# A-SHOJAEI/adverse-weather-semantic-segmentation-robustness-benchmark

Hardware: AMD Instinct MI355X
Metric: images/sec (1024x2048, 5 weather conds, ensemble eval) (higher is better)
Workload: dtype f32 (results float32; attention, gemm_1x1, winograd_3x3, segformer_head on 3xf16 split operands: 22-bit operands, f32 accumulate)

## Files before the change

### adverse_weather_semantic_segmentation_robustness_benchmark_amd/_native.py

```python
from __future__ import annotations

import ctypes as C
from pathlib import Path

import numpy as np
import torch

_PKG = Path(__file__).resolve().parent
LIB_PATH = _PKG / "libawseg_hip.so"

U8, I64 = 0, 1
COMBINE_WEIGHTED, COMBINE_MAXCONF, COMBINE_MEAN = 0, 1, 2
LOSS_CE, LOSS_FOCAL = 0, 1
ACT_NONE, ACT_RELU, ACT_GELU = 0, 1, 2
MAX_CLASSES = 32

c_i, c_i64, c_u64, c_f, c_d, c_p = C.c_int, C.c_int64, C.c_uint64, C.c_float, C.c_double, C.c_void_p

FOG_JOB = np.dtype([("image", "<i4"), ("_pad", "<i4"), ("beta", "<f8"), ("atmos", "<f8"), ("seed", "<u8")], align=True)
NIGHT_JOB = np.dtype([("image", "<i4"), ("_pad", "<i4"), ("brightness", "<f8"), ("intensity", "<f8"), ("seed", "<u8")], align=True)
PRIM_JOB = np.dtype([("image", "<i4"), ("prim_offset", "<i4"), ("prim_count", "<i4"), ("blur_ksize", "<i4"), ("intensity", "<f8")], align=True)
WEATHER_JOB = np.dtype([("kind", "<i4"), ("image", "<i4"), ("a", "<f8"), ("b", "<f8"), ("seed", "<u8"), ("prim_offset", "<i4"), ("prim_count", "<i4")], align=True)
WEATHER_CLEAN, WEATHER_FOG, WEATHER_RAIN, WEATHER_SNOW, WEATHER_NIGHT = 0, 1, 2, 3, 4
assert FOG_JOB.itemsize == 32 and NIGHT_JOB.itemsize == 32 and PRIM_JOB.itemsize == 24 and WEATHER_JOB.itemsize == 40
# ... 97 lines not shown
    "awseg_depth_eval_stats": (c_i, [c_p, c_p, c_i, c_i, c_i, c_i, c_i, c_p, c_p, c_f, c_p, c_p, c_i, c_p]),
    "awseg_ensemble_failure_stats": (c_i, [c_p, c_p, c_p, c_i64, c_i, c_i64, c_i, c_p, c_p, c_p, c_i, c_p, c_p, c_i, c_p]),
    "awseg_failure_stats": (c_i, [c_p, c_i64, c_i, c_i64, c_p, c_i, c_p, c_p, c_i, c_p]),
    "awseg_boundary_workspace": (c_i64, [c_i64, c_i, c_i, c_i, c_i]),
    "awseg_boundary_stats": (c_i, [c_p, c_p, c_i, c_i, c_i64, c_i, c_i, c_i, c_p, c_i, c_p, c_p, c_i, c_p, c_p, c_p]),
    "awseg_segment_workspace": (c_i64, [c_i64, c_i, c_i]),
    "awseg_segment_stats": (c_i, [c_p, c_p, c_i, c_i, c_i64, c_i, c_i, c_i, c_p, c_i, c_p, c_p, c_p, c_i, c_p, c_p, c_p, c_p, c_p]),
    "awseg_frame_iou_workspace": (c_i64, [c_i64, c_i, c_i64]),
    "awseg_frame_iou_counts": (c_i, [c_p, c_p, c_i, c_i, c_i64, c_i64, c_i, c_p, c_p, c_i64, c_p, c_p, c_p]),
    "awseg_bootstrap_counts": (c_i, [c_p, c_p, c_i64, c_i64, c_i64, c_i64, c_u64, c_i64, c_i64, c_p, c_p, c_p]),
    "awseg_change_strata": (c_i, [c_p, c_p, c_i, c_i64, c_i, c_i64, c_p, c_p, c_p, c_i, c_p, c_p, c_p]),
    "awseg_strata_workspace": (c_i64, [c_i64, c_i, c_i64, c_i]),
    "awseg_stratified_stats": (c_i, [c_p, c_p, c_i, c_i, c_p, c_i, c_p, c_i, c_p, c_i64, c_i64, c_i, c_p, c_p, c_i, c_p, c_p, c_p]),
    "awseg_image_quality_workspace": (c_i64, [c_i64, c_i, c_i64, c_i64]),
    "awseg_image_quality": (c_i, [c_p, c_p, c_i, c_i64, c_i, c_i64, c_i64, c_p, c_p, c_p, c_p, c_f, c_f, c_p, c_p, c_i, c_p, c_p, c_p]),
}

EXTENSION_SIGNATURES = {
    "awseg_restore_header_hash": (C.c_uint64, []),
    "awseg_dehaze_workspace": (c_i64, [c_i64, c_i64, c_i64]),
    "awseg_dehaze": (c_i, [c_p, c_i64, c_i, c_i64, c_i64, c_p, c_p, c_i, c_f, c_f, c_f, c_i, c_p, c_p, c_p, c_p, c_i, c_p, c_p]),
    "awseg_dehaze_guided_workspace": (c_i64, [c_i64, c_i64, c_i64]),
    "awseg_dehaze_guided": (c_i, [c_p, c_i64, c_i, c_i64, c_i64, c_p, c_p, c_i, c_f, c_f, c_f, c_i, c_f, c_p, c_p, c_p, c_p, c_p, c_p, c_i,
                                  c_p, c_p]),
    "awseg_relight_workspace": (c_i64, [c_i64, c_i, c_i]),
    "awseg_relight": (c_i, [c_p, c_i64, c_i, c_i64, c_i64, c_p, c_p, c_i, c_i, c_f, c_f, c_i, c_p, c_p, c_p, c_p, c_i, c_p, c_p]),
    "awseg_deocclude_workspace": (c_i64, [c_i64, c_i64, c_i64]),
    "awseg_deocclude": (c_i, [c_p, c_i64, c_i, c_i64, c_i64, c_p, c_p, c_i, c_f, c_f, c_i, c_p, c_p, c_p, c_p, c_i, c_p, c_p]),
    "awseg_weather_estimate_workspace": (c_i64, [c_i64]),
    "awseg_weather_estimate": (c_i, [c_p, c_i64, c_i, c_i64, c_i64, c_p, c_p, c_i, c_f, c_f, c_f, c_f, c_f, c_f, c_p, c_p, c_p, c_p, c_i,
                                     c_p, c_p]),
}


class AwsegError(RuntimeError):
    pass


_lib = None


def lib() -> C.CDLL:
    global _lib
    if _lib is None:
        if not LIB_PATH.exists():
            raise AwsegError(
                f"{LIB_PATH} is missing: build it with `python -m "
                "adverse_weather_semantic_segmentation_robustness_benchmark_amd.csrc.build` "
                "(there is no CPU fallback for the HIP hot path)")
        handle = C.CDLL(str(LIB_PATH))
        for table in (SIGNATURES, EXTENSION_SIGNATURES):
            for name, (res, args) in table.items():
                fn = getattr(handle, name)
                fn.restype, fn.argtypes = res, args
        header = LIB_PATH.parent.parent / "include" / "awseg.h"
        built = int(handle.awseg_header_hash())
        if built and header.exists():
            from .csrc.build import header_hash
            if built != header_hash():
                raise AwsegError(f"{LIB_PATH} was built from another include/awseg.h than the one beside it (ABI drift): rebuild it with "
                                 "`python -m adverse_weather_semantic_segmentation_robustness_benchmark_amd.csrc.build`")
        extension = header.with_name("awseg_restore.h")
        built = int(handle.awseg_restore_header_hash())
        if built and extension.exists():
            from .csrc.build import RESTORE_HEADER, header_hash
            if built != header_hash(RESTORE_HEADER):
                raise AwsegError(f"{LIB_PATH} was built from another include/awseg_restore.h than the one beside it (ABI drift): rebuild "
                                 "it with `python -m adverse_weather_semantic_segmentation_robustness_benchmark_amd.csrc.build`")
        _lib = handle
    return _lib


def check(rc: int, what: str) -> None:
    if rc != 0:
        msg = lib().awseg_error_string(rc)
        raise AwsegError(f"{what} failed with code {rc}: {msg.decode() if msg else '?'}")


launch_hook = None


def call(name: str, *args) -> None:
    fn = getattr(lib(), name)
    rc = fn(*args) if launch_hook is None else launch_hook(name, lambda: fn(*args), args)
    check(rc, name)


def try_call(name: str, *args, allow=(-2,)) -> int:
    fn = getattr(lib(), name)
    rc = fn(*args) if launch_hook is None else launch_hook(name, lambda: fn(*args), args)
    if rc != 0 and rc not in allow:
        check(rc, name)
    return rc


def ptr(t):
    if t is None:
        return None
    if not t.is_cuda:
        raise AwsegError("awseg kernels take device (HIP) tensors only; got a CPU tensor — no CPU fallback exists")
    if not t.is_contiguous():
# ... 49 lines not shown
```

### adverse_weather_semantic_segmentation_robustness_benchmark_amd/csrc/build.py

```python
from __future__ import annotations

import os
import shutil
import subprocess
import sys
from concurrent.futures import ThreadPoolExecutor
from pathlib import Path

CSRC = Path(__file__).resolve().parent
PKG = CSRC.parent
LIB = PKG / "libawseg_hip.so"
SOURCES = ["core.hip", "metrics.hip", "weather.hip", "loss.hip", "heads.hip", "backbone.hip", "depth.hip", "wino.hip", "gemm.hip", "attn.hip", "gemm_split.hip", "gemm_split3.hip", "wino_split.hip", "depthfuse.hip", "mixffn.hip", "dwtrain.hip", "bntrain.hip", "smallops.hip", "calib.hip", "consistency.hip", "deptheval.hip", "failure.hip", "boundary.hip", "bootstrap.hip", "strata.hip", "quality.hip", "segments.hip", "weightgrid.hip", "dehaze.hip", "dehaze_guided.hip", "relight.hip", "deocclude.hip", "estimate.hip"]
ARCH = "gfx950"
HEADER = PKG.parent / "include" / "awseg.h"
RESTORE_HEADER = PKG.parent / "include" / "awseg_restore.h"


def header_hash(path: Path = HEADER) -> int:
    import hashlib
    return int(hashlib.sha256(path.read_bytes()).hexdigest()[:15], 16)


EXTRA_FLAGS = {"attn.hip": ["-DAWSEG_ATTN_SPLIT_WAVES=" + os.environ.get("AWSEG_ATTN_SPLIT_WAVES", "2")], "wino.hip": ["-fno-slp-vectorize"], "wino_split.hip": ["-fno-slp-vectorize"],
               "core.hip": ["-DAWSEG_HEADER_HASH=0x%xULL" % header_hash()],
               "dehaze.hip": ["-DAWSEG_RESTORE_HEADER_HASH=0x%xULL" % header_hash(RESTORE_HEADER)]}


def hipcc() -> str:
    for cand in (os.environ.get("HIPCC"), "/opt/rocm/bin/hipcc", shutil.which("hipcc")):
        if cand and Path(cand).exists():
            return cand
    raise RuntimeError("hipcc not found (need ROCm's hipcc to build libawseg_hip.so)")


def _flags():
    return [f"--offload-arch={ARCH}", "-O3", "-std=c++17", "-fPIC", "-ffp-contract=off",
            "-fvisibility=hidden", "-Wall", "-Wno-unused-function", "-Wno-inline-asm"]


STAMP = PKG / "libawseg_hip.flags"


def _flag_stamp() -> str:
    return repr((_flags(), sorted(EXTRA_FLAGS.items()), SOURCES))


def needs_build() -> bool:
    if not LIB.exists():
        return True
    if not STAMP.exists() or STAMP.read_text() != _flag_stamp():
        return True
    t = LIB.stat().st_mtime
    deps = [CSRC / s for s in SOURCES] + sorted(CSRC.glob("*.h")) + [HEADER, RESTORE_HEADER]
    return any(d.stat().st_mtime > t for d in deps)


def build(force: bool = False, verbose: bool = False) -> Path:
    if not force and not needs_build():
        return LIB
    cc = hipcc()
    objdir = CSRC / "build"
    objdir.mkdir(exist_ok=True)

    def compile_one(src):
        obj = objdir / (Path(src).stem + ".o")
        cmd = [cc, *_flags(), *EXTRA_FLAGS.get(src, []), "-c", str(CSRC / src), "-o", str(obj)]
        if verbose:
            print(" ".join(cmd))
        subprocess.check_call(cmd)
        return obj

    with ThreadPoolExecutor(max_workers=min(4, len(SOURCES))) as ex:
        objs = list(ex.map(compile_one, SOURCES))
    tmp = LIB.with_suffix(".so.tmp")
    rocm_lib = str(Path(cc).resolve().parent.parent / "lib")
    subprocess.check_call([cc, f"--offload-arch={ARCH}", "-shared", "-fPIC", "-o", str(tmp), *map(str, objs),
                           f"-L{rocm_lib}", "-lhipblaslt", f"-Wl,-rpath,{rocm_lib}"])
    os.replace(tmp, LIB)
    STAMP.write_text(_flag_stamp())
    return LIB


if __name__ == "__main__":
    print(build(force="--force" in sys.argv, verbose=True))
```

### adverse_weather_semantic_segmentation_robustness_benchmark_amd/models/fused.py

```python
from __future__ import annotations

import contextlib
import os
from typing import List

import torch
import torch.nn as nn
import torch.nn.functional as F

from .. import _native as N
from .. import ops

CL = torch.channels_last


def _pair(v):
    return (v, v) if isinstance(v, int) else tuple(v)


def _versions(*tensors):
    return tuple((t.data_ptr(), t._version) for t in tensors if t is not None)


DERIVED = ("wsplit", "wbf16", "wsplit_small", "kvsplit", "proj_pieces", "stemrows")
# ... 178 lines not shown
            scale = bn.weight * inv
            sh = bn.bias - bn.running_mean * scale
            if conv.bias is not None:
                sh = sh + conv.bias * scale
            return patch_weights(conv, scale), sh.contiguous()
        w2, sh = cached(conv, "patch", [conv.weight, conv.bias, bn.weight, bn.bias, bn.running_mean, bn.running_var], build)
        return conv_gemm_nhwc(nhwc_view(x), conv, w2, sh, act).permute(0, 3, 1, 2)
    if _is_winograd(conv) and act in (N.ACT_NONE, N.ACT_RELU):
        y = conv3x3_winograd_bn(nhwc_view(x), conv, bn, act, None if residual is None else nhwc_view(residual))
        return y.permute(0, 3, 1, 2)
    y = F.conv2d(x, w, None, conv.stride, conv.padding, conv.dilation, conv.groups)
    if not y.is_contiguous(memory_format=CL):
        y = y.contiguous(memory_format=CL)
    ops.bias_act_nhwc_(y.permute(0, 2, 3, 1), shift, None if residual is None else nhwc_view(residual), act)
    return y


STEM_ROWS = os.environ.get("AWSEG_STEM_ROWS", "1") != "0"
_stem_pad = {}
_stem_scope = None


@contextlib.contextmanager
def stem_scope():
    global _stem_scope
    prev, _stem_scope = _stem_scope, {}
    try:
        yield
    finally:
        _stem_scope = prev


def stem_image_ok(x: torch.Tensor) -> bool:
    return STEM_ROWS and ops.GEMM_SPLIT and x.is_cuda and x.dtype == torch.float32 and x.dim() == 4 and x.shape[1] <= 4 and ops.PRECISION != "bf16"


def stem_image(x: torch.Tensor) -> torch.Tensor:
    B, C, H, W = x.shape
    wp_any = max(W + 3, ((W + 6 - 7) // 2) * 2 + 8, ((W + 6 - 7) // 4) * 4 + 8)
    skey = (x.data_ptr(), tuple(x.shape), tuple(x.stride()))
    xp = _stem_scope.get(skey) if _stem_scope is not None else None
    if xp is None:
        key = (str(x.device), B, H, W, C, wp_any)
        xp = _stem_pad.get(key)
        if xp is None:
            _stem_pad.clear()
            xp = _stem_pad[key] = torch.zeros(B, H, wp_any, 4, dtype=torch.float32, device=x.device)
        if x.stride(3) == 1 and x.stride(2) >= W and min(x.stride()) >= 0:
            ops.stem_image_fill(x, xp)
        else:
            xp[:, :, 3:3 + W, :C] = x.permute(0, 2, 3, 1)
        if _stem_scope is not None:
            _stem_scope[skey] = xp
    return xp


def _stem_rows(x: torch.Tensor, conv: nn.Conv2d, w: torch.Tensor, bias: torch.Tensor = None):
    st = conv.stride[0]
    if not (STEM_ROWS and ops.GEMM_SPLIT and x.is_cuda and x.dtype == torch.float32 and conv.kernel_size == (7, 7) and conv.stride in ((2, 2), (4, 4))
            and conv.padding == (3, 3) and conv.dilation == (1, 1) and conv.groups == 1 and conv.in_channels <= 4
            and (conv.out_channels % 64 == 0 or 8 <= conv.out_channels < 64) and ops.PRECISION != "bf16"):
        return None
    B, C, H, W = x.shape
    wo = (W + 6 - 7) // st + 1
    wp = max(W + 3, (wo - 1) * st + 8)
    xp = stem_image(x)
    assert wp <= xp.shape[2]
    ws = cached(conv, "stemrows", [w], lambda: ops.gemm_split_weights(ops.stem_rows_weights(w)))
    return ops.conv_rows_gemm_split(xp, ws, bias, N.ACT_NONE, 7, st, 3, wo)


def _bottleneck_tail_dual(out: torch.Tensor, y: torch.Tensor, blk):
    c3, cd, bn3, bnd = blk.conv3, blk.downsample[0], blk.bn3, blk.downsample[1]
    if not (ops.DUAL_TAIL and ops.GEMM_SPLIT and ops.PRECISION != "bf16" and out.is_cuda and out.dtype == torch.float32
            and c3.kernel_size == (1, 1) and cd.kernel_size == (1, 1) and c3.stride == (1, 1) and c3.groups == 1 and cd.groups == 1
            and cd.stride[0] == cd.stride[1] and cd.padding == (0, 0) and c3.padding == (0, 0)
            and c3.in_channels % 32 == 0 and cd.in_channels % 32 == 0 and isinstance(bnd, nn.BatchNorm2d)):
        return None
    ol, yl = nhwc_view(out), nhwc_view(y)
    B, Ho, Wo, k1 = ol.shape
    _, H, W, k2 = yl.shape
    st = cd.stride[0]
    if (H - 1) // st + 1 != Ho or (W - 1) // st + 1 != Wo:
        return None
    n = c3.out_channels

    def build():
        w3, b3 = folded_conv_bn(c3, bn3)
        wd, bd = folded_conv_bn(cd, bnd)
        return ops.gemm_split_weights(torch.cat([w3.reshape(n, k1), wd.reshape(n, k2)], dim=1).contiguous()), (b3 + bd).contiguous()
    ws, bias = cached(blk, "dualtail", [c3.weight, bn3.weight, bn3.bias, bn3.running_mean, bn3.running_var,
                                        cd.weight, bnd.weight, bnd.bias, bnd.running_mean, bnd.running_var], build)
    y2 = ops.gemm_split_dual(ol.view(B * Ho * Wo, k1), yl if st > 1 else yl.view(B * H * W, k2), ws, bias, N.ACT_RELU, stride=st if st > 1 else 0)
    return None if y2 is None else y2.view(B, Ho, Wo, n).permute(0, 3, 1, 2)


@torch.no_grad()
def resnet_features(enc, x: torch.Tensor, stem_feature: bool = False) -> List[torch.Tensor]:
    feats = [x]
    if stem_feature:
        x = x.contiguous(memory_format=CL)
        feats = [x]
        y = conv_bn_act(x, enc.conv1, enc.bn1, N.ACT_RELU)
        feats.append(y)
        y = enc.maxpool(y)
    else:
        w, shift = folded_conv_bn(enc.conv1, enc.bn1)
        y = _stem_rows(x, enc.conv1, w)
        y = y.permute(0, 3, 1, 2) if y is not None else F.conv2d(x.contiguous(memory_format=CL), w, None, enc.conv1.stride, enc.conv1.padding)
        mp = enc.maxpool
        if (y.is_cuda and y.dtype == torch.float32 and y.is_contiguous(memory_format=CL) and y.shape[1] % 4 == 0
                and _pair(mp.kernel_size) == (3, 3) and _pair(mp.stride) == (2, 2) and _pair(mp.padding) == (1, 1)
                and _pair(mp.dilation) == (1, 1) and not mp.ceil_mode):
            y = ops.maxpool3x3s2_nhwc(nhwc_view(y), shift=shift).permute(0, 3, 1, 2)
        else:
            y = mp(y)
            if not y.is_contiguous(memory_format=CL):
                y = y.contiguous(memory_format=CL)
            ops.bias_act_nhwc_(y.permute(0, 2, 3, 1), shift, None, N.ACT_RELU)
        feats.append(None)
    for layer in (enc.layer1, enc.layer2, enc.layer3, enc.layer4):
        for blk in layer:
            out = conv_bn_act(y, blk.conv1, blk.bn1, N.ACT_RELU)
            out = conv_bn_act(out, blk.conv2, blk.bn2, N.ACT_RELU)
            if blk.downsample is not None:
                y2 = _bottleneck_tail_dual(out, y, blk)
                if y2 is not None:
                    y = y2
                    continue
            idn = y if blk.downsample is None else conv_bn_act(y, blk.downsample[0], blk.downsample[1], N.ACT_NONE)
            scratch = not any(idn is f for f in feats)
            y = conv_bn_act(out, blk.conv3, blk.bn3, N.ACT_RELU, residual=idn, residual_is_scratch=scratch)
        feats.append(y)
    return feats


@torch.no_grad()
def separable_bn_relu(x: torch.Tensor, sep, bn: nn.BatchNorm2d) -> torch.Tensor:
    dwc, pwc = sep[0], sep[1]
    xl = nhwc_view(x)
    B, H, W, C = xl.shape
    d = ops.dwconv3x3_nhwc(xl, dw_taps(dwc), None, N.ACT_NONE, dilation=dwc.dilation[0])
    w, shift = folded_conv_bn(pwc, bn)
    w2 = w.view(w.shape[0], C)
# ... 25 lines not shown
    if lin.bias is None or not tok.is_contiguous():
        return tok + F.linear(x2, lin.weight, lin.bias).view_as(tok)
    t2 = tok.view(-1, tok.shape[-1])
    ops.gemm_bias_act(x2, lin.weight, lin.bias, N.ACT_NONE, residual=t2, out=t2, w_split=split_weights(lin, lin.weight, x2.shape[0]))
    return tok


def _kv_packed(kv: torch.Tensor, a) -> torch.Tensor:
    kp, vp = a.k_proj, a.v_proj
    wkv, bkv = cached(a, "kvpack", [kp.weight, kp.bias, vp.weight, vp.bias],
                      lambda: (torch.cat([kp.weight, vp.weight]).contiguous(), torch.cat([kp.bias, vp.bias]).contiguous()))
    c = kv.shape[-1]
    m = kv.numel() // c
    if ops.gemm_wants_bf16(m, 2 * c, c) or ops.gemm_wants_split(m, 2 * c, c):
        y = ops.gemm_bias_act(kv.view(m, c), wkv, bkv, N.ACT_NONE, w_split=split_weights(a, wkv, m))
    else:
        ws = cached(a, "kvsplit", (wkv,), lambda: ops.gemm_split_weights(wkv))
        y = ops.gemm_bias_act(kv.view(m, c), wkv, bkv, N.ACT_NONE, w_split=ws, split=True)
    return y.view(*kv.shape[:-1], 2 * c)


@torch.no_grad()
def mit_features_nhwc(seg, x: torch.Tensor) -> torch.Tensor:
    if not hasattr(seg, "stages"):
        return seg(x).last_hidden_state.permute(0, 2, 3, 1).contiguous()
    t = x
    tok = None
    for st in seg.stages:
        pe = st.patch_embeddings
        if _is_patch_gemm(pe.proj) and pe.proj.bias is not None:
            w2 = cached(pe.proj, "patch", [pe.proj.weight], lambda: patch_weights(pe.proj))
            y = conv_gemm_nhwc(nhwc_view(t), pe.proj, w2, pe.proj.bias, N.ACT_NONE)
        else:
            y = _stem_rows(t, pe.proj, pe.proj.weight, pe.proj.bias) if pe.proj.bias is not None else None
            if y is None:
                w = cached(pe.proj, "wcl", [pe.proj.weight], lambda: pe.proj.weight.contiguous(memory_format=CL))
                y = nhwc_view(F.conv2d(t.contiguous(memory_format=CL), w, pe.proj.bias, pe.proj.stride, pe.proj.padding))
        tok = _ln(y, pe.layer_norm)
        B, H, W, C = tok.shape
        for blk in st.blocks:
            a = blk.attention
            hcur = _ln(tok, blk.layernorm_before)
            q = _linear(hcur, a.q_proj)
            if a.sequence_reduction_ratio > 1:
                sr = a.sequence_reduction
                src = sr.sequence_reduction
                if _is_patch_gemm(src) and src.bias is not None:
                    w2 = cached(src, "patch", [src.weight], lambda: patch_weights(src))
                    kv = conv_gemm_nhwc(hcur, src, w2, src.bias, N.ACT_NONE)
                else:
                    wsr = cached(src, "wcl", [src.weight], lambda: src.weight.contiguous(memory_format=CL))
                    kv = nhwc_view(F.conv2d(hcur.permute(0, 3, 1, 2), wsr, src.bias, src.stride))
                kv = _ln(kv, sr.layer_norm)
            else:
                kv = hcur
            nh, d = a.num_attention_heads, a.head_dim
            nkv = kv.shape[1] * kv.shape[2]
            if (d == 32 and nkv % 32 == 0 and ops.KV_PACKED and kv.is_cuda and kv.dtype == torch.float32 and C % 8 == 0
                    and a.k_proj.bias is not None and a.v_proj.bias is not None and kv.is_contiguous()):
                o = ops.attention_d32_packed_kv(q.view(B, H * W, C), _kv_packed(kv, a).view(B, nkv, 2 * C), nh, a.scaling).view(B * H * W, C)
            elif d == 32 and nkv % 32 == 0:
                k, v = _linear(kv, a.k_proj), _linear(kv, a.v_proj)
                o = ops.attention_d32(q.view(B, H * W, C), k.reshape(B, nkv, C), v.reshape(B, nkv, C), nh, a.scaling).view(B * H * W, C)
            else:
                k, v = _linear(kv, a.k_proj), _linear(kv, a.v_proj)
                qq, kk, vv = (t_.view(B, -1, nh, d).transpose(1, 2) for t_ in (q.view(B, H * W, C), k.reshape(B, -1, C), v.reshape(B, -1, C)))
                if ops.PRECISION == "bf16":
# ... 29 lines not shown
```

### adverse_weather_semantic_segmentation_robustness_benchmark_amd/ops.py

```python
from __future__ import annotations

import math
import os

import ctypes as C
from typing import Optional, Sequence

import numpy as np
import torch

from . import _native as N

IMAGENET_MEAN = np.array([0.485, 0.456, 0.406], dtype=np.float32)
IMAGENET_STD = np.array([0.229, 0.224, 0.225], dtype=np.float32)
NIGHT_GAINS = np.array([0.8, 0.85, 1.2], dtype=np.float32)
CONDITIONS = ("clean", "fog", "rain", "snow", "night")


def gaussian_taps(sigma: float = 2.0, truncate: float = 4.0) -> np.ndarray:
    radius = int(truncate * float(sigma) + 0.5)
    x = np.arange(-radius, radius + 1)
    phi = np.exp(-0.5 / (sigma * sigma) * x ** 2)
    return phi / phi.sum()

# ... 1907 lines not shown
    ATTENTION_SPLIT, GEMM_SPLIT, WINO_SPLIT = bool(state["attention"]), bool(state["gemm_1x1"]), bool(state["winograd_3x3"])
    HEAD_SPLIT = bool(state.get("segformer_head", HEAD_SPLIT))


def maxpool3x3s2_nhwc(x_nhwc: torch.Tensor, shift: Optional[torch.Tensor] = None) -> torch.Tensor:
    x = x_nhwc.contiguous()
    b, h, w, c = x.shape
    out = torch.empty(b, (h - 1) // 2 + 1, (w - 1) // 2 + 1, c, dtype=torch.float32, device=x.device)
    if shift is not None:
        N.call("awseg_maxpool3x3s2_bias_relu_nhwc", N.ptr(x), b, h, w, c, N.ptr(shift.contiguous()), N.ptr(out), N.stream())
    else:
        N.call("awseg_maxpool3x3s2_nhwc", N.ptr(x), b, h, w, c, N.ptr(out), N.stream())
    return out


def upsample_bilinear(x: torch.Tensor, size, align_corners: bool) -> torch.Tensor:
    b, c, h, w = x.shape
    H, W = int(size[0]), int(size[1])
    if not (x.is_contiguous() or (STRIDED_UPSAMPLE and W % 4 == 0 and 3 * w < W and 3 * h < H and all(s_ >= 0 for s_ in x.stride()))):
        x = x.contiguous()
    out = torch.empty(b, c, H, W, dtype=torch.float32, device=x.device)
    sb, sc, sy, sx = (c * h * w, h * w, w, 1) if x.is_contiguous() else x.stride()
    N.call("awseg_upsample_bilinear_strided", N.ptr_strided(x), b, c, h, w, sb, sc, sy, sx, H, W, int(bool(align_corners)), N.ptr(out), N.stream())
    return out


def stem_image_fill(x: torch.Tensor, image: torch.Tensor) -> None:
    b, c, h, w = x.shape
    if x.stride(3) != 1:
        x = x.contiguous()
    N.call("awseg_stem_image", N.ptr_strided(x), b, c, h, w, x.stride(0), x.stride(1), x.stride(2), N.ptr(image), image.shape[2], N.stream())


def rowdot_sigmoid(x: torch.Tensor, w: torch.Tensor, bias: Optional[torch.Tensor], sigmoid: bool = True) -> torch.Tensor:
    x, w = x.contiguous(), w.contiguous().view(-1)
    out = torch.empty(x.shape[0], dtype=torch.float32, device=x.device)
    N.call("awseg_rowdot_sigmoid", N.ptr(x), x.shape[0], x.shape[1], N.ptr(w), N.ptr(bias), int(bool(sigmoid)), N.ptr(out), N.stream())
    return out


def aspp_pool_branch(mean: torch.Tensor, w1: torch.Tensor, b1: torch.Tensor, w2: torch.Tensor, b2: Optional[torch.Tensor]) -> torch.Tensor:
    mean, w1, b1, w2 = mean.contiguous(), w1.contiguous(), b1.contiguous(), w2.contiguous()
    b, cin = mean.shape
    cmid, cout = w1.shape[0], w2.shape[0]
    ws = torch.empty(int(N.lib().awseg_aspp_pool_branch_workspace(b, cmid)), dtype=torch.uint8, device=mean.device)
    out = torch.empty(b, cout, dtype=torch.float32, device=mean.device)
    N.call("awseg_aspp_pool_branch", N.ptr(mean), b, cin, N.ptr(w1), N.ptr(b1), cmid, N.ptr(w2), N.ptr(None if b2 is None else b2.contiguous()),
           cout, N.ptr(ws), N.ptr(out), N.stream())
    return out


def depth_upsample_combine(d1: torch.Tensor, d2_low: torch.Tensor, weights: Optional[torch.Tensor]):
    d1, d2_low = d1.contiguous(), d2_low.contiguous()
    b, _, H, W = d1.shape
    h, w = d2_low.shape[-2:]
    d2_full, d = torch.empty_like(d1), torch.empty_like(d1)
    N.call("awseg_depth_upsample_combine", N.ptr(d1), N.ptr(d2_low), b, h, w, H, W, N.ptr(None if weights is None else weights.contiguous()),
           N.ptr(d2_full), N.ptr(d), N.stream())
    return d2_full, d


def layernorm_rows(x: torch.Tensor, gamma: torch.Tensor, beta: torch.Tensor, eps: float) -> torch.Tensor:
    x = x.contiguous()
    c = x.shape[-1]
    out = torch.empty_like(x)
    N.call("awseg_layernorm_rows", N.ptr(x), x.numel() // c, c, N.ptr(gamma.contiguous()), N.ptr(beta.contiguous()), float(eps),
# ... 3 lines not shown
```

Measured before the change: 234.6.

## Add tiled MFMA 7x7 stem kernel fusing conv with 3x3 maxpool

```diff
diff --git a/adverse_weather_semantic_segmentation_robustness_benchmark_amd/_native.py b/adverse_weather_semantic_segmentation_robustness_benchmark_amd/_native.py
--- a/adverse_weather_semantic_segmentation_robustness_benchmark_amd/_native.py
+++ b/adverse_weather_semantic_segmentation_robustness_benchmark_amd/_native.py
@@ -153,6 +153,12 @@
                                      c_p, c_p]),
 }
 
+STEM_SIGNATURES = {
+    "awseg_stem_header_hash": (C.c_uint64, []),
+    "awseg_stem7x7_split": (c_i, [c_p, c_i, c_i, c_i, c_i, c_i64, c_i64, c_i64, c_i, c_i, c_p, c_p, c_p, c_i, c_p]),
+    "awseg_stem7x7_plan": (c_i, [c_i, c_i, c_i, c_i, c_i, c_p, c_p]),
+}
+
 
 class AwsegError(RuntimeError):
     pass
@@ -170,7 +176,7 @@
                 "adverse_weather_semantic_segmentation_robustness_benchmark_amd.csrc.build` "
                 "(there is no CPU fallback for the HIP hot path)")
         handle = C.CDLL(str(LIB_PATH))
-        for table in (SIGNATURES, EXTENSION_SIGNATURES):
+        for table in (SIGNATURES, EXTENSION_SIGNATURES, STEM_SIGNATURES):
             for name, (res, args) in table.items():
                 fn = getattr(handle, name)
                 fn.restype, fn.argtypes = res, args
@@ -188,6 +194,13 @@
             if built != header_hash(RESTORE_HEADER):
                 raise AwsegError(f"{LIB_PATH} was built from another include/awseg_restore.h than the one beside it (ABI drift): rebuild "
                                  "it with `python -m adverse_weather_semantic_segmentation_robustness_benchmark_amd.csrc.build`")
+        stem = header.with_name("awseg_stem.h")
+        built = int(handle.awseg_stem_header_hash())
+        if built and stem.exists():
+            from .csrc.build import STEM_HEADER, header_hash
+            if built != header_hash(STEM_HEADER):
+                raise AwsegError(f"{LIB_PATH} was built from another include/awseg_stem.h than the one beside it (ABI drift): rebuild "
+                                 "it with `python -m adverse_weather_semantic_segmentation_robustness_benchmark_amd.csrc.build`")
         _lib = handle
     return _lib
 
diff --git a/adverse_weather_semantic_segmentation_robustness_benchmark_amd/csrc/build.py b/adverse_weather_semantic_segmentation_robustness_benchmark_amd/csrc/build.py
--- a/adverse_weather_semantic_segmentation_robustness_benchmark_amd/csrc/build.py
+++ b/adverse_weather_semantic_segmentation_robustness_benchmark_amd/csrc/build.py
@@ -10,10 +10,11 @@
 CSRC = Path(__file__).resolve().parent
 PKG = CSRC.parent
 LIB = PKG / "libawseg_hip.so"
-SOURCES = ["core.hip", "metrics.hip", "weather.hip", "loss.hip", "heads.hip", "backbone.hip", "depth.hip", "wino.hip", "gemm.hip", "attn.hip", "gemm_split.hip", "gemm_split3.hip", "wino_split.hip", "depthfuse.hip", "mixffn.hip", "dwtrain.hip", "bntrain.hip", "smallops.hip", "calib.hip", "consistency.hip", "deptheval.hip", "failure.hip", "boundary.hip", "bootstrap.hip", "strata.hip", "quality.hip", "segments.hip", "weightgrid.hip", "dehaze.hip", "dehaze_guided.hip", "relight.hip", "deocclude.hip", "estimate.hip"]
+SOURCES = ["core.hip", "metrics.hip", "weather.hip", "loss.hip", "heads.hip", "backbone.hip", "depth.hip", "wino.hip", "gemm.hip", "attn.hip", "gemm_split.hip", "gemm_split3.hip", "stem.hip", "wino_split.hip", "depthfuse.hip", "mixffn.hip", "dwtrain.hip", "bntrain.hip", "smallops.hip", "calib.hip", "consistency.hip", "deptheval.hip", "failure.hip", "boundary.hip", "bootstrap.hip", "strata.hip", "quality.hip", "segments.hip", "weightgrid.hip", "dehaze.hip", "dehaze_guided.hip", "relight.hip", "deocclude.hip", "estimate.hip"]
 ARCH = "gfx950"
 HEADER = PKG.parent / "include" / "awseg.h"
 RESTORE_HEADER = PKG.parent / "include" / "awseg_restore.h"
+STEM_HEADER = PKG.parent / "include" / "awseg_stem.h"
 
 
 def header_hash(path: Path = HEADER) -> int:
@@ -23,7 +24,8 @@
 
 EXTRA_FLAGS = {"attn.hip": ["-DAWSEG_ATTN_SPLIT_WAVES=" + os.environ.get("AWSEG_ATTN_SPLIT_WAVES", "2")], "wino.hip": ["-fno-slp-vectorize"], "wino_split.hip": ["-fno-slp-vectorize"],
                "core.hip": ["-DAWSEG_HEADER_HASH=0x%xULL" % header_hash()],
-               "dehaze.hip": ["-DAWSEG_RESTORE_HEADER_HASH=0x%xULL" % header_hash(RESTORE_HEADER)]}
+               "dehaze.hip": ["-DAWSEG_RESTORE_HEADER_HASH=0x%xULL" % header_hash(RESTORE_HEADER)],
+               "stem.hip": ["-DAWSEG_STEM_HEADER_HASH=0x%xULL" % header_hash(STEM_HEADER)]}
 
 
 def hipcc() -> str:
@@ -51,7 +53,7 @@
     if not STAMP.exists() or STAMP.read_text() != _flag_stamp():
         return True
     t = LIB.stat().st_mtime
-    deps = [CSRC / s for s in SOURCES] + sorted(CSRC.glob("*.h")) + [HEADER, RESTORE_HEADER]
+    deps = [CSRC / s for s in SOURCES] + sorted(CSRC.glob("*.h")) + [HEADER, RESTORE_HEADER, STEM_HEADER]
     return any(d.stat().st_mtime > t for d in deps)
 
 
diff --git a/adverse_weather_semantic_segmentation_robustness_benchmark_amd/csrc/stem.hip b/adverse_weather_semantic_segmentation_robustness_benchmark_amd/csrc/stem.hip
--- /dev/null
+++ b/adverse_weather_semantic_segmentation_robustness_benchmark_amd/csrc/stem.hip
@@ -0,0 +1,372 @@
+#include "awseg_common.h"
+#include "../../include/awseg_stem.h"
+
+namespace {
+
+typedef float f32x16 __attribute__((ext_vector_type(16)));
+typedef _Float16 h8 __attribute__((ext_vector_type(8)));
+typedef unsigned u32x2 __attribute__((ext_vector_type(2)));
+typedef unsigned u32x4 __attribute__((ext_vector_type(4)));
+
+constexpr float kStScale0 = 16.0f;
+constexpr int kStExp0 = -4;
+constexpr float kStBig = 2048.0f;
+constexpr float kStSmall = 0.0078125f;
+constexpr int kStWaves = 4;
+constexpr int kStSteps = 14;
+constexpr unsigned kOob = 0x80000000u;
+
+__device__ __forceinline__ float st_pow2(int e) { return __builtin_bit_cast(float, (unsigned)(127 + e) << 23); }
+
+__device__ __forceinline__ void st_split2(float a, float b, float s, unsigned& hi, unsigned& lo)
+{
+    asm("v_fma_mixlo_f16 %0, %2, %4, 0\n\t"
+        "v_fma_mixhi_f16 %0, %3, %4, 0\n\t"
+        "v_fma_mixlo_f16 %1, %2, %4, -%0 op_sel_hi:[0,0,1]\n\t"
+        "v_fma_mixhi_f16 %1, %3, %4, -%0 op_sel:[0,0,1] op_sel_hi:[0,0,1]\n\t"
+        "s_nop 1"
+        : "=&v"(hi), "=&v"(lo) : "v"(a), "v"(b), "s"(s));
+}
+
+struct st_args {
+    const float* x; int64_t sb; int sc, sy;
+    int B, C, H, W, Ho, Wo;
+    int Ro, Co;
+    const uint16_t* w3; const unsigned* trailer;
+    const float* bias; float* out; int N;
+    int nsx, nsg, seg_rows, units;
+    unsigned x_bytes;
+};
+
+template <int S, int MT> struct st_geo {
+    static constexpr int PW = 31 * S + 8;
+    static constexpr int GR = S * MT;
+    static constexpr int RING = 3 * GR;
+    static constexpr int NM = PW / 64, REM = PW % 64;
+    static constexpr int PLANE = RING * PW * 8;
+    static constexpr int WAVE_LDS = 2 * PLANE;
+    static_assert((MT - 1) * S + 6 < 2 * GR, "a chunk reads two ring groups");
+    static_assert(REM * 4 <= 64 && PW % 2 == 0, "window layout");
+};
+template <int S, int MT, int NT> constexpr int st_lds() { return NT * kStSteps * 2 * 1024 + kStWaves * st_geo<S, MT>::WAVE_LDS; }
+
+template <int S, int MT, int NT, bool POOL>
+__global__ __launch_bounds__(64 * kStWaves)
+void stem7x7_split_kernel(st_args a)
+{
+    using G = st_geo<S, MT>;
+    constexpr int PW = G::PW, GR = G::GR, RING = G::RING, NM = G::NM, REM = G::REM;
+    extern __shared__ __attribute__((aligned(16))) unsigned char smem[];
+    const int tid = threadIdx.x, lane = tid & 63, wave = tid >> 6;
+    const int hk = lane >> 5, li = lane & 31;
+
+    for (int d = tid; d < kStSteps * 2 * NT * 64; d += 64 * kStWaves) {
+        const int l = d & 63, j = (d >> 6) % NT, qh = (d >> 6) / NT, half = qh & 1, q = qh >> 1;
+        const int n = 32 * j + (l & 31), t = q >> 1, ks = q & 1;
+        const u32x4 v = *reinterpret_cast<const u32x4*>(a.w3 + ((int64_t)(t * 64 + n) * 64 + half * 32 + (2 * ks + (l >> 5)) * 8));
+        *reinterpret_cast<u32x4*>(smem + d * 16) = v;
+    }
+    __syncthreads();
+    const unsigned char* sW = smem;
+    unsigned char* sHi = smem + NT * kStSteps * 2 * 1024 + wave * G::WAVE_LDS;
+    unsigned char* sLo = sHi + G::PLANE;
+    const int we = (int)a.trailer[1];
+    const int fragA = (S * li + 2 * hk) * 8;
+
+    float bv[NT];
+#pragma unroll
+    for (int j = 0; j < NT; ++j) bv[j] = (a.bias && 32 * j + li < a.N) ? a.bias[32 * j + li] : 0.f;
+
+    for (int u = blockIdx.x * kStWaves + wave; u < a.units; u += gridDim.x * kStWaves) {
+        const int sx = u % a.nsx, ut = u / a.nsx, sg = ut % a.nsg, b = ut / a.nsg;
+        const int r0 = sg * a.seg_rows, r1 = r0 + a.seg_rows < a.Ro ? r0 + a.seg_rows : a.Ro;
+        const int q0 = sx * (POOL ? 15 : 32);
+        const int cy0 = POOL ? 2 * r0 - 1 : r0, cx0 = POOL ? 2 * q0 - 1 : q0;
+        const int nrows = POOL ? 2 * (r1 - r0) + 1 : r1 - r0;
+        const int nchunks = (nrows + MT - 1) / MT;
+        const int iy0 = cy0 * S - 3, ix0 = cx0 * S - 3;
+        const bool colsin = cx0 >= 0 && cx0 + 32 <= a.Wo;
+        const __amdgpu_buffer_rsrc_t rsrc = __builtin_amdgcn_make_buffer_rsrc((void*)(a.x + (int64_t)b * a.sb), 0, (int)a.x_bytes, 0x00020000);
+        unsigned vm[NM][4], vl;
+#pragma unroll
+        for (int m = 0; m < NM; ++m)
+#pragma unroll
+            for (int c = 0; c < 4; ++c) {
+                const int ix = ix0 + 64 * m + lane;
+                vm[m][c] = (c < a.C && ix >= 0 && ix < a.W) ? (unsigned)((c * a.sc + ix) * 4) : kOob;
+            }
+        {
+            const int c = lane / REM, ix = ix0 + 64 * NM + lane % REM;
+            vl = (lane < 4 * REM && c < a.C && ix >= 0 && ix < a.W) ? (unsigned)((c * a.sc + ix) * 4) : kOob;
+        }
+        const int lrem = (64 * NM + lane % REM) * 8 + (lane / REM) * 2;
+
+        float sxs = kStScale0;
+        int xe = kStExp0;
+        for (int pass = 0; pass < 2; ++pass) {
+            float amax = 0.f;
+            float gm[GR][NM][4], gl[GR];
+            auto load = [&](int gi) {
+#pragma unroll
+                for (int r = 0; r < GR; ++r) {
+                    const int iy = iy0 + GR * gi + r;
+                    const bool ok = iy >= 0 && iy < a.H;
+                    const unsigned so = ok ? (unsigned)(iy * a.sy * 4) : 0u;
+#pragma unroll
+                    for (int m = 0; m < NM; ++m)
+#pragma unroll
+                        for (int c = 0; c < 4; ++c)
+                            gm[r][m][c] = __builtin_bit_cast(float, __builtin_amdgcn_raw_buffer_load_b32(rsrc, ok ? vm[m][c] : kOob, so, 0));
+                    gl[r] = __builtin_bit_cast(float, __builtin_amdgcn_raw_buffer_load_b32(rsrc, ok ? vl : kOob, so, 0));
+                }
+            };
+            auto write = [&](int gi) {
+                const int rb = GR * (gi % 3);
+#pragma unroll
+                for (int r = 0; r < GR; ++r) {
+                    const int rowb = (rb + r) * PW * 8;
+#pragma unroll
+                    for (int m = 0; m < NM; ++m) {
+                        unsigned h0, l0, h1, l1;
+                        st_split2(gm[r][m][0], gm[r][m][1], sxs, h0, l0);
+                        st_split2(gm[r][m][2], gm[r][m][3], sxs, h1, l1);
+                        amax = __builtin_fmaxf(__builtin_fmaxf(amax, __builtin_fabsf(gm[r][m][0])), __builtin_fabsf(gm[r][m][1]));
+                        amax = __builtin_fmaxf(__builtin_fmaxf(amax, __builtin_fabsf(gm[r][m][2])), __builtin_fabsf(gm[r][m][3]));
+                        *reinterpret_cast<u32x2*>(sHi + rowb + (64 * m + lane) * 8) = u32x2{h0, h1};
+                        *reinterpret_cast<u32x2*>(sLo + rowb + (64 * m + lane) * 8) = u32x2{l0, l1};
+                    }
+                    unsigned h, l;
+                    st_split2(gl[r], 0.f, sxs, h, l);
+                    amax = __builtin_fmaxf(amax, __builtin_fabsf(gl[r]));
+                    if (lane < 4 * REM) {
+                        *reinterpret_cast<uint16_t*>(sHi + rowb + lrem) = (uint16_t)h;
+                        *reinterpret_cast<uint16_t*>(sLo + rowb + lrem) = (uint16_t)l;
+                    }
+                }
+            };
+
+            const int oe = we + xe;
+            const int oe1 = oe / 2, oe2 = oe - oe1;
+            const float os1 = st_pow2(oe1 < -126 ? -126 : (oe1 > 127 ? 127 : oe1)), os2 = st_pow2(oe2 < -126 ? -126 : (oe2 > 127 ? 127 : oe2));
+            float cur[NT][8];
+#pragma unroll
+            for (int j = 0; j < NT; ++j)
+#pragma unroll
+                for (int i = 0; i < 8; ++i) cur[j][i] = -__builtin_inff();
+
+            load(0); write(0);
+            load(1); write(1);
+            for (int g = 0; g < nchunks; ++g) {
+                const bool more = g + 2 <= nchunks;
+                if (more) load(g + 2);
+                f32x16 acc[MT][NT];
+#pragma unroll
+                for (int mt = 0; mt < MT; ++mt)
+#pragma unroll
+                    for (int j = 0; j < NT; ++j)
+#pragma unroll
+                        for (int r = 0; r < 16; ++r) acc[mt][j][r] = 0.f;
+                const int rb = GR * (g % 3);
+#pragma unroll
+                for (int ky = 0; ky < 7; ++ky) {
+                    int rowb[MT];
+#pragma unroll
+                    for (int mt = 0; mt < MT; ++mt) {
+                        int r = rb + S * mt + ky;
+                        r = r >= RING ? r - RING : r;
+                        rowb[mt] = r * PW * 8 + fragA;
+                    }
+#pragma unroll
+                    for (int ks = 0; ks < 2; ++ks) {
+                        const int q = 2 * ky + ks;
+                        h8 Bh[NT], Bl[NT];
+#pragma unroll
+                        for (int j = 0; j < NT; ++j) {
+                            Bh[j] = *reinterpret_cast<const h8*>(sW + ((q * 2 + 0) * NT + j) * 1024 + lane * 16);
+                            Bl[j] = *reinterpret_cast<const h8*>(sW + ((q * 2 + 1) * NT + j) * 1024 + lane * 16);
+                        }
+#pragma unroll
+                        for (int mt = 0; mt < MT; ++mt) {
+                            const h8 Ah = *reinterpret_cast<const h8*>(sHi + rowb[mt] + ks * 32);
+                            const h8 Al = *reinterpret_cast<const h8*>(sLo + rowb[mt] + ks * 32);
+#pragma unroll
+                            for (int j = 0; j < NT; ++j) {
+                                acc[mt][j] = __builtin_amdgcn_mfma_f32_32x32x16_f16(Ah, Bh[j], acc[mt][j], 0, 0, 0);
+                                acc[mt][j] = __builtin_amdgcn_mfma_f32_32x32x16_f16(Ah, Bl[j], acc[mt][j], 0, 0, 0);
+                                acc[mt][j] = __builtin_amdgcn_mfma_f32_32x32x16_f16(Al, Bh[j], acc[mt][j], 0, 0, 0);
+                            }
+                        }
+                    }
+                }
+
+#pragma unroll
+                for (int mt = 0; mt < MT; ++mt) {
+                    const int y = MT * g + mt;
+                    if (y >= nrows) break;
+                    const int cy = cy0 + y;
+                    if (!POOL) {
+                        float* orow = a.out + ((((int64_t)b * a.Ho + cy) * a.Wo + cx0 + 4 * hk) * a.N + li);
+#pragma unroll
+                        for (int j = 0; j < NT; ++j) {
+                            const bool nin = 32 * j + li < a.N;
+#pragma unroll
+                            for (int r = 0; r < 16; ++r) {
+                                const int dx = 8 * (r >> 2) + (r & 3);
+                                float vv = acc[mt][j][r] * os1 * os2;
+                                vv = vv + bv[j];
+                                vv = __builtin_fmaxf(vv, -__builtin_inff());
+                                if (nin && (colsin || cx0 + 4 * hk + dx < a.Wo)) orow[dx * a.N + 32 * j] = vv;
+                            }
+                        }
+                        continue;
+                    }
+                    const bool rowin = cy >= 0 && cy < a.Ho;
+                    float hp[NT][8];
+#pragma unroll
+                    for (int j = 0; j < NT; ++j) {
+                        float v[16];
+#pragma unroll
+                        for (int r = 0; r < 16; ++r) {
+                            const int cx = cx0 + 8 * (r >> 2) + 4 * hk + (r & 3);
+                            v[r] = (colsin || (cx >= 0 && cx < a.Wo)) ? acc[mt][j][r] : -__builtin_inff();
+                            v[r] = rowin ? v[r] : -__builtin_inff();
+                        }
+#pragma unroll
+                        for (int q = 0; q < 4; ++q) {
+                            const float send = hk ? v[4 * q] : v[q < 3 ? 4 * (q + 1) : 0];
+                            const float recv = __shfl_xor(send, 32, 64);
+                            hp[j][2 * q] = __builtin_fmaxf(__builtin_fmaxf(v[4 * q], v[4 * q + 1]), v[4 * q + 2]);
+                            hp[j][2 * q + 1] = __builtin_fmaxf(__builtin_fmaxf(v[4 * q + 2], v[4 * q + 3]), recv);
+                        }
+                    }
+                    if (y & 1) {
+#pragma unroll
+                        for (int j = 0; j < NT; ++j)
+#pragma unroll
+                            for (int i = 0; i < 8; ++i) cur[j][i] = __builtin_fmaxf(cur[j][i], hp[j][i]);
+                    } else {
+                        if (y > 0) {
+                            const int pr = r0 + y / 2 - 1;
+                            float* orow = a.out + ((((int64_t)b * a.Ro + pr) * a.Co + q0 + 2 * hk) * a.N + li);
+#pragma unroll
+                            for (int j = 0; j < NT; ++j) {
+                                const bool nin = 32 * j + li < a.N;
+#pragma unroll
+                                for (int i = 0; i < 8; ++i) {
+                                    const int dq = 4 * (i >> 1) + (i & 1);
+                                    float rr = __builtin_fmaxf(cur[j][i], hp[j][i]) * os1 * os2;
+                                    rr = rr + 0.f;
+                                    rr = __builtin_fmaxf(rr, -__builtin_inff());
+                                    rr = rr + bv[j];
+                                    rr = rr > 0.f ? rr : 0.f;
+                                    if (nin && 2 * hk + dq < 15 && q0 + 2 * hk + dq < a.Co) orow[dq * a.N + 32 * j] = rr;
+                                }
+                            }
+                        }
+#pragma unroll
+                        for (int j = 0; j < NT; ++j)
+#pragma unroll
+                            for (int i = 0; i < 8; ++i) cur[j][i] = hp[j][i];
+                    }
+                }
+                if (more) write(g + 2);
+            }
+
+            if (pass == 1) break;
+            const bool big = __ballot(amax >= kStBig) != 0ull;
+            const bool small = __ballot(amax >= kStSmall) == 0ull;
+            if (!big && !small) break;
+            float mxf = amax;
+#pragma unroll
+            for (int o = 32; o > 0; o >>= 1) mxf = __builtin_fmaxf(mxf, __shfl_xor(mxf, o, 64));
+            const unsigned mx = __builtin_bit_cast(unsigned, mxf);
+            constexpr unsigned kSmallBits = __builtin_bit_cast(unsigned, kStSmall);
+            if (!(big || (mx >= 0x00800000u && mx < kSmallBits))) break;
+            const int ex = (int)(mx >> 23) & 0xff;
+            if (ex == 0xff) break;
+            xe = ex - 127 - 13;
+            xe = xe < -127 ? -127 : xe;
+            sxs = st_pow2(-xe);
+        }
+    }
+}
+
+struct st_plan { int ho, wo, ro, co, nsx, nsg, seg_rows, units, blocks; };
+bool st_make_plan(int batch, int height, int width, int stride, int mode, int cus, st_plan& p)
+{
+    p.ho = (height + 6 - 7) / stride + 1; p.wo = (width + 6 - 7) / stride + 1;
+    if (height < 1 || width < 1 || p.ho < 1 || p.wo < 1) return false;
+    p.ro = mode == AWSEG_STEM_POOL ? (p.ho + 2 - 3) / 2 + 1 : p.ho;
+    p.co = mode == AWSEG_STEM_POOL ? (p.wo + 2 - 3) / 2 + 1 : p.wo;
+    const int strip = mode == AWSEG_STEM_POOL ? 15 : 32;
+    p.nsx = (p.co + strip - 1) / strip;
+    const int64_t cols = (int64_t)batch * p.nsx, waves = (int64_t)cus * kStWaves;
+    int64_t nsg = 2 * waves / cols;
+    const int min_rows = mode == AWSEG_STEM_POOL ? 4 : 8;
+    if (nsg < 1) nsg = 1;
+    int seg = (int)((p.ro + nsg - 1) / nsg);
+    if (seg < min_rows) seg = min_rows;
+    p.seg_rows = seg;
+    p.nsg = (p.ro + seg - 1) / seg;
+    const int64_t units = cols * p.nsg;
+    if (units > 0x7fffffff) return false;
+    p.units = (int)units;
+    const int64_t blocks = (units + kStWaves - 1) / kStWaves;
+    p.blocks = (int)(blocks < cus ? blocks : cus);
+    return true;
+}
+
+}
+
+#ifndef AWSEG_STEM_HEADER_HASH
+#define AWSEG_STEM_HEADER_HASH 0ULL
+#endif
+AWSEG_API uint64_t awseg_stem_header_hash(void) { return AWSEG_STEM_HEADER_HASH; }
+
+AWSEG_API int awseg_stem7x7_plan(int batch, int height, int width, int stride, int mode, int* units, int* blocks)
+{
+    st_plan p;
+    if (batch < 1 || (stride != 2 && stride != 4) || (mode != AWSEG_STEM_POOL && mode != AWSEG_STEM_PLAIN) || !units || !blocks) return AWSEG_EINVAL;
+    if (!st_make_plan(batch, height, width, stride, mode, awseg_cu_count(), p)) return AWSEG_ERANGE;
+    *units = p.units; *blocks = p.blocks;
+    return 0;
+}
+
+AWSEG_API int awseg_stem7x7_split(const float* x, int batch, int channels, int height, int width, int64_t stride_b, int64_t stride_c,
+                                  int64_t stride_y, int stride, int mode, const uint16_t* w_split, const float* bias, float* out, int n,
+                                  awseg_stream_t stream)
+{
+    if (batch == 0) return 0;
+    if (!x || !w_split || !out || batch < 0 || channels < 1 || height < 1 || width < 1 || stride_b < 0 || stride_c < 0 || stride_y < width) return AWSEG_EINVAL;
+    if ((stride != 2 && stride != 4) || (mode != AWSEG_STEM_POOL && mode != AWSEG_STEM_PLAIN)) return AWSEG_EINVAL;
+    if (channels > 4 || !(n == 64 || (n >= 8 && n < 64)) || (mode == AWSEG_STEM_POOL && stride != 2)) return AWSEG_ERANGE;
+    if (((uintptr_t)x & 3) || ((uintptr_t)w_split & 15)) return AWSEG_EALIGN;
+    const int64_t extent = ((int64_t)(channels - 1) * stride_c + (int64_t)(height - 1) * stride_y + width) * 4;
+    if (extent > 0x7fffffff) return AWSEG_ERANGE;
+    st_plan p;
+    if (!st_make_plan(batch, height, width, stride, mode, awseg_cu_count(), p)) return AWSEG_ERANGE;
+    st_args a;
+    a.x = x; a.sb = stride_b; a.sc = (int)stride_c; a.sy = (int)stride_y;
+    a.B = batch; a.C = channels; a.H = height; a.W = width; a.Ho = p.ho; a.Wo = p.wo; a.Ro = p.ro; a.Co = p.co;
+    const int64_t k = 224;
+    a.trailer = reinterpret_cast<const unsigned*>(w_split + 2 * (int64_t)n * k);
+    a.w3 = w_split + 2 * (int64_t)n * k + 8;
+    a.bias = bias; a.out = out; a.N = n;
+    a.nsx = p.nsx; a.nsg = p.nsg; a.seg_rows = p.seg_rows; a.units = p.units;
+    a.x_bytes = (unsigned)extent;
+#define ST_GO(S_, MT_, NT_, POOL_)                                                                                                      \
+    do {                                                                                                                               \
+        auto kf = stem7x7_split_kernel<S_, MT_, NT_, POOL_>;                                                                           \
+        constexpr int lds = st_lds<S_, MT_, NT_>();                                                                                    \
+        hipError_t e = hipFuncSetAttribute(reinterpret_cast<const void*>(kf), hipFuncAttributeMaxDynamicSharedMemorySize, lds);         \
+        if (e != hipSuccess) return (int)e;                                                                                            \
+        hipLaunchKernelGGL(kf, dim3((unsigned)p.blocks), dim3(64 * kStWaves), lds, awseg_s(stream), a);                                 \
+    } while (0)
+    const bool two = n > 32;
+    if (mode == AWSEG_STEM_POOL) { if (two) ST_GO(2, 3, 2, true); else ST_GO(2, 3, 1, true); }
+    else if (stride == 2) { if (two) ST_GO(2, 3, 2, false); else ST_GO(2, 3, 1, false); }
+    else { if (two) ST_GO(4, 1, 2, false); else ST_GO(4, 1, 1, false); }
+#undef ST_GO
+    AWSEG_LAUNCH_CHECK();
+    return 0;
+}
diff --git a/adverse_weather_semantic_segmentation_robustness_benchmark_amd/models/fused.py b/adverse_weather_semantic_segmentation_robustness_benchmark_amd/models/fused.py
--- a/adverse_weather_semantic_segmentation_robustness_benchmark_amd/models/fused.py
+++ b/adverse_weather_semantic_segmentation_robustness_benchmark_amd/models/fused.py
@@ -234,7 +234,9 @@
 
 
 def stem_image_ok(x: torch.Tensor) -> bool:
-    return STEM_ROWS and ops.GEMM_SPLIT and x.is_cuda and x.dtype == torch.float32 and x.dim() == 4 and x.shape[1] <= 4 and ops.PRECISION != "bf16"
+    if not (STEM_ROWS and ops.GEMM_SPLIT and x.is_cuda and x.dtype == torch.float32 and x.dim() == 4 and x.shape[1] <= 4 and ops.PRECISION != "bf16"):
+        return False
+    return not (STEM_TILE and _rows_kernel_takes(x, 4, 32))
 
 
 def stem_image(x: torch.Tensor) -> torch.Tensor:
@@ -272,6 +274,28 @@
     return ops.conv_rows_gemm_split(xp, ws, bias, N.ACT_NONE, 7, st, 3, wo)
 
 
+STEM_TILE = os.environ.get("AWSEG_STEM_TILE", "1") != "0"
+
+
+def _rows_kernel_takes(x: torch.Tensor, st: int, n: int) -> bool:
+    B, C, H, W = x.shape
+    m = B * ((H - 1) // st + 1) * ((W - 1) // st + 1)
+    wp_any = max(W + 3, ((W + 6 - 7) // 2) * 2 + 8, ((W + 6 - 7) // 4) * 4 + 8)
+    cus = torch.cuda.get_device_properties(x.device).multi_processor_count
+    return n <= 64 and (m + 127) // 128 >= cus // 2 and B * H * wp_any * 16 <= 0x7fffffff
+
+
+def _stem_tile(x: torch.Tensor, conv: nn.Conv2d, w: torch.Tensor, bias: torch.Tensor, pool: bool):
+    st = conv.stride[0]
+    if not (STEM_TILE and STEM_ROWS and ops.GEMM_SPLIT and x.is_cuda and x.dtype == torch.float32 and conv.kernel_size == (7, 7)
+            and conv.stride in ((2, 2), (4, 4)) and conv.padding == (3, 3) and conv.dilation == (1, 1) and conv.groups == 1
+            and conv.in_channels <= 4 and 8 <= conv.out_channels <= 64 and ops.PRECISION != "bf16" and (st == 2 or not pool)
+            and _rows_kernel_takes(x, st, conv.out_channels)):
+        return None
+    ws = cached(conv, "stemrows", [w], lambda: ops.gemm_split_weights(ops.stem_rows_weights(w)))
+    return ops.stem7x7_split(x, ws, bias, st, pool)
+
+
 def _bottleneck_tail_dual(out: torch.Tensor, y: torch.Tensor, blk):
     c3, cd, bn3, bnd = blk.conv3, blk.downsample[0], blk.bn3, blk.downsample[1]
     if not (ops.DUAL_TAIL and ops.GEMM_SPLIT and ops.PRECISION != "bf16" and out.is_cuda and out.dtype == torch.float32
@@ -308,10 +332,17 @@
         y = enc.maxpool(y)
     else:
         w, shift = folded_conv_bn(enc.conv1, enc.bn1)
-        y = _stem_rows(x, enc.conv1, w)
+        mp = enc.maxpool
+        pool_ok = (_pair(mp.kernel_size) == (3, 3) and _pair(mp.stride) == (2, 2) and _pair(mp.padding) == (1, 1)
+                   and _pair(mp.dilation) == (1, 1) and not mp.ceil_mode)
+        y = _stem_tile(x, enc.conv1, w, shift, True) if pool_ok else None
+        pooled = y is not None
+        if not pooled:
+            y = _stem_rows(x, enc.conv1, w)
         y = y.permute(0, 3, 1, 2) if y is not None else F.conv2d(x.contiguous(memory_format=CL), w, None, enc.conv1.stride, enc.conv1.padding)
-        mp = enc.maxpool
-        if (y.is_cuda and y.dtype == torch.float32 and y.is_contiguous(memory_format=CL) and y.shape[1] % 4 == 0
+        if pooled:
+            pass
+        elif (y.is_cuda and y.dtype == torch.float32 and y.is_contiguous(memory_format=CL) and y.shape[1] % 4 == 0
                 and _pair(mp.kernel_size) == (3, 3) and _pair(mp.stride) == (2, 2) and _pair(mp.padding) == (1, 1)
                 and _pair(mp.dilation) == (1, 1) and not mp.ceil_mode):
             y = ops.maxpool3x3s2_nhwc(nhwc_view(y), shift=shift).permute(0, 3, 1, 2)
@@ -403,7 +434,9 @@
             w2 = cached(pe.proj, "patch", [pe.proj.weight], lambda: patch_weights(pe.proj))
             y = conv_gemm_nhwc(nhwc_view(t), pe.proj, w2, pe.proj.bias, N.ACT_NONE)
         else:
-            y = _stem_rows(t, pe.proj, pe.proj.weight, pe.proj.bias) if pe.proj.bias is not None else None
+            y = _stem_tile(t, pe.proj, pe.proj.weight, pe.proj.bias, False) if pe.proj.bias is not None else None
+            if y is None:
+                y = _stem_rows(t, pe.proj, pe.proj.weight, pe.proj.bias) if pe.proj.bias is not None else None
             if y is None:
                 w = cached(pe.proj, "wcl", [pe.proj.weight], lambda: pe.proj.weight.contiguous(memory_format=CL))
                 y = nhwc_view(F.conv2d(t.contiguous(memory_format=CL), w, pe.proj.bias, pe.proj.stride, pe.proj.padding))
diff --git a/adverse_weather_semantic_segmentation_robustness_benchmark_amd/ops.py b/adverse_weather_semantic_segmentation_robustness_benchmark_amd/ops.py
--- a/adverse_weather_semantic_segmentation_robustness_benchmark_amd/ops.py
+++ b/adverse_weather_semantic_segmentation_robustness_benchmark_amd/ops.py
@@ -1963,6 +1963,33 @@
     N.call("awseg_stem_image", N.ptr_strided(x), b, c, h, w, x.stride(0), x.stride(1), x.stride(2), N.ptr(image), image.shape[2], N.stream())
 
 
+STEM_POOL, STEM_PLAIN = 1, 0
+
+
+def stem7x7_split(x: torch.Tensor, w_split: torch.Tensor, bias: Optional[torch.Tensor], stride: int, pool: bool) -> torch.Tensor:
+    b, c, h, w = x.shape
+    n, k = w_split.shape[1], w_split.shape[2]
+    if k != 224:
+        raise N.AwsegError("stem7x7_split: weights must be the [N, 224] matrix of stem_rows_weights")
+    if not _split_weights_intact(w_split, n, k):
+        raise N.AwsegError("w_split lost its 16-byte trailer (weight exponent): pass the tensor gemm_split_weights returned, not a copy")
+    if x.stride(3) != 1 or x.stride(2) < w or min(x.stride()) < 0:
+        x = x.contiguous()
+    ho, wo = (h - 1) // stride + 1, (w - 1) // stride + 1
+    if pool:
+        ho, wo = (ho - 1) // 2 + 1, (wo - 1) // 2 + 1
+    out = torch.empty(b, ho, wo, n, dtype=torch.float32, device=x.device)
+    N.call("awseg_stem7x7_split", N.ptr_strided(x), b, c, h, w, x.stride(0), x.stride(1), x.stride(2), stride, STEM_POOL if pool else STEM_PLAIN,
+           N.ptr(w_split), N.ptr(None if bias is None else bias.contiguous()), N.ptr(out), n, N.stream())
+    return out
+
+
+def stem7x7_plan(batch: int, height: int, width: int, stride: int, pool: bool):
+    units, blocks = C.c_int(0), C.c_int(0)
+    N.call("awseg_stem7x7_plan", batch, height, width, stride, STEM_POOL if pool else STEM_PLAIN, C.byref(units), C.byref(blocks))
+    return units.value, blocks.value
+
+
 def rowdot_sigmoid(x: torch.Tensor, w: torch.Tensor, bias: Optional[torch.Tensor], sigmoid: bool = True) -> torch.Tensor:
     x, w = x.contiguous(), w.contiguous().view(-1)
     out = torch.empty(x.shape[0], dtype=torch.float32, device=x.device)
diff --git a/include/awseg_stem.h b/include/awseg_stem.h
--- /dev/null
+++ b/include/awseg_stem.h
@@ -0,0 +1,23 @@
+#ifndef AWSEG_STEM_H
+#define AWSEG_STEM_H
+
+#include "awseg.h"
+
+#ifdef __cplusplus
+extern "C" {
+#endif
+
+uint64_t awseg_stem_header_hash(void);
+
+#define AWSEG_STEM_PLAIN 0
+#define AWSEG_STEM_POOL  1
+int awseg_stem7x7_split(const float* x, int batch, int channels, int height, int width, int64_t stride_b, int64_t stride_c,
+                        int64_t stride_y, int stride, int mode, const uint16_t* w_split, const float* bias, float* out, int n,
+                        awseg_stream_t stream);
+int awseg_stem7x7_plan(int batch, int height, int width, int stride, int mode, int* units, int* blocks);
+
+#ifdef __cplusplus
+}
+#endif
+
+#endif
```

After: 227.5. -3.0%, worse.
